# Jakoebly/marl-sc

Hardware: AMD Instinct MI355X
Metric: env-steps/sec (agents×envs×steps) at 1/2/4/8 MI355X; CPU ref same host (higher is better)
Workload: dtype int32 state, u64 PCG64, f64 rewards, f32 obs; 1 GPU; InventoryEnvironment.step x 32768 envs/GPU, 8 agents x 64 regions x 5 SKUs (BASELINE configs[2]; configs[3] when N>1); n_envs_per_gpu=32768, agents=8, regions=64, skus=5, episode_length=100, obs_dim_local=34, obs_normalization=meanstd_custom, parallelism=env-shard x1

## Files before the change

### marl-sc_amd/csrc/demand_v3.hip

```cpp
#include <hip/hip_runtime.h>

#include "demand_common.hpp"

namespace msc {

#ifdef MSC_PROF
__device__ unsigned long long g_prof_v3[8];
#endif

template <int K, int G, bool EA>
__global__ __launch_bounds__(BS * (1 + G)) __attribute__((amdgpu_waves_per_eu(MSC_DEM_WPE))) void demand_v3_kernel(
    const DevEnv* __restrict__ dp, EaLaunch ea) {
  const EnvConst& c = dp->c;
  const EnvState& s = dp->s;
  constexpr int NV = Rec<K>::NV;
  extern __shared__ __attribute__((aligned(16))) double v3lds[];
  __shared__ int more[2];
  double* ring = v3lds;
  int32_t* rdv = reinterpret_cast<int32_t*>(v3lds + BS * USLOTS);
  const int wave = (int)(threadIdx.x / BS), lane = (int)(threadIdx.x % BS);
  const int64_t E = c.E;
  const int64_t vlane = (int64_t)blockIdx.x * BS + lane;
  int64_t e = vlane;
  int slot = 0, ea_k = 0;
  bool valid = vlane < E;
  if constexpr (EA) {
    valid = vlane < (int64_t)ea.nslots * E;
    ea_k = valid ? (int)(vlane / E) : 0;
    e = valid ? vlane - (int64_t)ea_k * E : 0;
    slot = (ea.slot0 + ea_k) % c.ea_S;
  }
  double* myring = ring + lane;
  int ea_cnt_new = 0;
  uint32_t ea_p0 = 0;
  int ea_n0 = 0;
  if constexpr (EA) {
    if (valid && ea.t0 > 0) {
      ea_p0 = s.ea_pos[((int64_t)slot * c.T + (ea.t0 - 1)) * E + e];
      ea_n0 = s.ea_off[((int64_t)slot * (c.T + 1) + ea.t0) * E + e];
    }
  }
  auto start_rng = [&]() -> Pcg64 {
    if constexpr (EA) {
      uint32_t root;
      if (ea.t0 == 0) {
        root = ea_root(c, s, ea, e, ea_k, slot, ea_cnt_new);
      } else {
        const uint32_t w2[2] = {s.orig_root[e], (uint32_t)(s.ea_cnt[(int64_t)slot * E + e] - 1)};
        root = ss_u32(w2, 2);
      }
      Pcg64 r;
      pcg_seed_child(r, root, 2);
      if (ea_p0) pcg_advance(r, (uint64_t)ea_p0);
      return r;
    } else {
      return load_rng(s, 0, e, E);
    }
  };

  if (wave > 0) {
    if (MSC_GEN_PRIO > 0) __builtin_amdgcn_s_setprio(MSC_GEN_PRIO);
    const int g = wave - 1;
    uint64_t th = 0, tl = 0, ih = 0, il = 1;
    if (valid) {
      Pcg64 rg = start_rng();
      for (int j = 0; j <= g; j++) pcg_step(rg);
      th = rg.s_hi;
      tl = rg.s_lo;
      ih = rg.i_hi;
      il = rg.i_lo;
    }
    uint64_t mh = PCG_MUL_HI, ml = PCG_MUL_LO, ch = ih, cl = il;
    if constexpr (G > 1) pcg_jump_coeffs(G, ih, il, mh, ml, ch, cl);
    int pg = g;
    GenLane gl = gen_lane(th, tl, ch, cl);
    auto gen_to = [&](int target) {
      while (pg < target) {
        const double u = gen_uniform(gl);
        const int sl = pg & (UCAP - 1);
        myring[sl * BS] = u;
        myring[(sl < UD - 1 ? sl + UCAP : USLOTS - 1) * BS] = u;
        gen_advance<G>(gl);
        pg += G;
      }
    };
    int tgt = UCAP;
    if (valid) gen_to(UCAP);
    __syncthreads();
    for (int ci = 0;; ci++) {
      const int rdp = rdv[(ci & 1) * BS + lane];
      tgt = unit_quota(tgt, rdp);
      if (valid) gen_to(tgt);
      __syncthreads();
      if (!more[ci & 1]) break;
      const int need = rdv[((ci + 1) & 1) * BS + lane] + UHS * UD;
      if (__ballot(valid && tgt < need) != 0) {
        tgt = tgt > need ? tgt : need;
        if (valid) gen_to(tgt);
        __syncthreads();
      }
    }
    return;
  }

  __builtin_amdgcn_s_setprio(MSC_PARSER_PRIO);
  Pcg64 r0{};
  if (valid) {
    r0 = start_rng();
    if constexpr (!EA) store_rng_pre(s, e, E, r0);
  }
  rdv[lane] = 0;
  static_assert(K <= UD, "a mask unit completes in one round");
  int qf = 0, mf = 0, of = valid ? 1 : 0, live = of;
  int r = 0, x = 0, left = 0, sq = 0, n = ea_n0, rd = 0, pend = 0;
  int tstep = EA ? ea.t0 : 0;
  unsigned mask = 0;
  const int cap = EA ? (int)c.ea_cap : c.order_cap;
  const int64_t vstride = EA ? 16 : E * 16;
  const int64_t rstride = (int64_t)NV * vstride;
  MSC_GLOBAL char* const recb = reinterpret_cast<MSC_GLOBAL char*>(
      gp(EA ? s.ea_rec + ((int64_t)slot * E + e) * c.ea_cap * NV : s.orders + e));
  decltype(s.ea_off) ea_offp = EA ? s.ea_off + (int64_t)slot * (c.T + 1) * E + e : nullptr;
  decltype(s.ea_pos) ea_posp = EA ? s.ea_pos + (int64_t)slot * c.T * E + e : nullptr;
  const int T_s = __builtin_amdgcn_readfirstlane(EA ? ea.t1 : c.T);
  __syncthreads();
  if constexpr (EA) {
    if (valid && ea.t0 == 0) {
      s.ea_cnt[(int64_t)slot * E + e] = ea_cnt_new;
      ea_offp[0] = 0;
    }
  }
  double thr_o = sgpr_d(c.uni_thr_o), thr_q = sgpr_d(c.uni_thr_q);
  asm volatile("" : "+v"(thr_o), "+v"(thr_q));
  const double thr_m = sgpr_d(c.uni_thr_m);
  const int R_s = __builtin_amdgcn_readfirstlane(c.R), cap_s = __builtin_amdgcn_readfirstlane(cap);
  const uint32_t rs32 = (uint32_t)__builtin_amdgcn_readfirstlane((uint32_t)rstride);
  auto rec_at = [&](int idx) -> MSC_GLOBAL char* { return recb + (int64_t)((uint64_t)(uint32_t)idx * rs32); };
  int ridx = (n < cap_s ? n : cap_s) - 1;
  double thr = thr_o, prod = 1.0;
  auto settle = [&]() {
    if (qf) {
      const int h = 1 + sq;
      MSC_GLOBAL char* fp = NV == 1 ? rec_at(ridx) + h * 2 : rec_at(ridx) + (int64_t)(h >> 3) * vstride + (h & 7) * 2;
      *reinterpret_cast<MSC_GLOBAL uint16_t*>(fp) = (uint16_t)(x > 1 ? x : 1);
    }
    const unsigned m2 = qf ? (mask & (mask - 1u)) : mask;
    const int has_q = (of ^ 1) & (m2 != 0u ? 1 : 0);
    const int left2 = (of ? x : left) - ((of | has_q) ^ 1);
    const int new_order = (has_q ^ 1) & (left2 > 0 ? 1 : 0);
    const int new_region = (has_q | new_order) ^ 1;
    int wrap = 0;
    if constexpr (EA) {
      if (new_region & (r + 1 == R_s ? 1 : 0)) {
        ea_offp[(int64_t)(tstep + 1) * E] = n;
        ea_posp[(int64_t)tstep * E] = ea_p0 + (uint32_t)rd;
        wrap = tstep + 1 < T_s ? 1 : 0;
        tstep += wrap;
      }
    }
    sq = __builtin_ctz(m2 | (1u << K));
    qf = has_q;
    mf = new_order;
    of = new_region & ((r + 1 < R_s ? 1 : 0) | wrap);
    live = qf | mf | of;
    thr = has_q ? thr_q : thr_o;
    mask = new_order ? 0u : m2;
    left = left2;
    n += new_order;
    ridx = (n < cap_s ? n : cap_s) - 1;
    if (new_order) {
      MSC_GLOBAL char* rp = rec_at(ridx);
#pragma unroll
      for (int j = 0; j < NV; j++)
        *reinterpret_cast<MSC_GLOBAL v4u*>(rp + (int64_t)j * vstride) = v4u{j == 0 ? (unsigned)r : 0u, 0u, 0u, 0u};
    }
    r = wrap ? 0 : r + new_region;
    prod = 1.0;
    x = 0;
  };
#ifdef MSC_PROF
  unsigned long long n_round = 0;
#endif
  int ptgt = UCAP, rd_start = 0;
  for (int ci = 0;; ci++) {
#pragma unroll 1
    for (int hs = 0; hs < UHS; hs++) {
      const double* rp = myring + (rd & (UCAP - 1)) * BS;
      double u[UD];
#pragma unroll
      for (int i = 0; i < UD; i++) u[i] = rp[i * BS];
      if (pend) settle();
      double p = prod;
      int ncont = 0;
      unsigned bits = 0;
#pragma unroll
      for (int i = 0; i < UD; i++) {
        p = p * u[i];
        ncont += p > thr ? 1 : 0;
        if (i < K) bits |= u[i] > thr_m ? 0u : (1u << i);
      }
      const int go = ncont >= UD ? 1 : 0;
      const int cons = mf ? K : (go ? UD : ncont + 1);
      mask = mf ? bits : mask;
      x += ncont;
      prod = p;
      rd += live ? cons : 0;
      pend = live & (mf | (go ^ 1));
#ifdef MSC_PROF
      n_round++;
#endif
    }
    const bool any = __ballot(live) != 0;
    rdv[((ci + 1) & 1) * BS + lane] = rd;
    if (lane == 0) more[ci & 1] = any ? 1 : 0;
    __syncthreads();
    if (!any) break;
    ptgt = unit_quota(ptgt, rd_start);
    const int need = rd + UHS * UD;
    if (__ballot(valid && ptgt < need) != 0) {
      ptgt = ptgt > need ? ptgt : need;
      __syncthreads();
    }
    rd_start = rd;
  }
#ifdef MSC_PROF
  if (lane == 0) {
    atomicAdd(&g_prof_v3[0], n_round);
    atomicAdd(&g_prof_v3[2], 1ull);
  }
#endif
  if (!valid) return;
  if constexpr (EA) {
    if (n > cap) atomicOr(s.err, ERR_ORDER_OVERFLOW);
    return;
  }
  pcg_advance(r0, (uint64_t)rd);
  store_rng(s, 0, e, E, r0);
  if (n > cap) {
    atomicOr(s.err, ERR_ORDER_OVERFLOW);
    n = cap;
  }
  s.n_orders[e] = n;
}

bool demand_v3_supported(const EnvConst& c) {
  return c.demand_uni != 0 && c.demand_ptrs == 0 && c.K >= 1 && c.K <= UD && c.K <= 8 &&
         (uint64_t)c.E * 32u < (1ull << 32);
}

template <int K>
static void launch_v3_k(const EnvConst& c, const DevEnv* d, hipStream_t st, const EaLaunch* ea) {
  constexpr int G = 3;
  if (ea) {
    hipLaunchKernelGGL((demand_v3_kernel<K, G, true>), dim3((unsigned)(((int64_t)ea->nslots * c.E + BS - 1) / BS)),
                       dim3(BS * (1 + G)), unit_lds_fixed(), st, d, *ea);
  } else {
    hipLaunchKernelGGL((demand_v3_kernel<K, G, false>), dim3((unsigned)((c.E + BS - 1) / BS)), dim3(BS * (1 + G)),
                       unit_lds_fixed(), st, d, EaLaunch{0, 0, 0, 0, 0, 0, 0});
  }
}

hipError_t launch_demand_v3(const EnvConst& c, const DevEnv* d, hipStream_t st, const EaLaunch* ea) {
  switch (c.K) {
    case 1: launch_v3_k<1>(c, d, st, ea); break;
    case 2: launch_v3_k<2>(c, d, st, ea); break;
    case 3: launch_v3_k<3>(c, d, st, ea); break;
    case 4: launch_v3_k<4>(c, d, st, ea); break;
    case 5: launch_v3_k<5>(c, d, st, ea); break;
    case 6: launch_v3_k<6>(c, d, st, ea); break;
    case 7: launch_v3_k<7>(c, d, st, ea); break;
    case 8: launch_v3_k<8>(c, d, st, ea); break;
    default: return hipErrorInvalidValue;
  }
  return hipGetLastError();
}

template <int G>
__global__ __launch_bounds__(BS) void gen_draws_kernel(const uint64_t* __restrict__ state, const uint64_t* __restrict__ inc,
                                                       int64_t n, uint64_t* __restrict__ out,
                                                       uint64_t* __restrict__ state_out) {
  if (blockIdx.x != 0) return;
  const int lane = (int)threadIdx.x;
  GenLane gl = gen_lane(state[2 * lane], state[2 * lane + 1], inc[2 * lane], inc[2 * lane + 1]);
  for (int64_t i = 0; i < n; i++) {
    out[(int64_t)lane * n + i] = (uint64_t)__double_as_longlong(gen_uniform(gl));
    gen_advance<G>(gl);
  }
  state_out[2 * lane] = gen_state_hi(gl);
  state_out[2 * lane + 1] = gen_state_lo(gl);
}

hipError_t launch_gen_draws(int G, const uint64_t* state, const uint64_t* inc, int64_t n, uint64_t* out,
                            uint64_t* state_out, hipStream_t st) {
  switch (G) {
    case 1: hipLaunchKernelGGL(gen_draws_kernel<1>, dim3(1), dim3(BS), 0, st, state, inc, n, out, state_out); break;
    case 2: hipLaunchKernelGGL(gen_draws_kernel<2>, dim3(1), dim3(BS), 0, st, state, inc, n, out, state_out); break;
    case 3: hipLaunchKernelGGL(gen_draws_kernel<3>, dim3(1), dim3(BS), 0, st, state, inc, n, out, state_out); break;
    case 5: hipLaunchKernelGGL(gen_draws_kernel<5>, dim3(1), dim3(BS), 0, st, state, inc, n, out, state_out); break;
    case 7: hipLaunchKernelGGL(gen_draws_kernel<7>, dim3(1), dim3(BS), 0, st, state, inc, n, out, state_out); break;
    default: return hipErrorInvalidValue;
  }
  return hipGetLastError();
}

#ifdef MSC_PROF
extern "C" int msc_debug_prof_v3(unsigned long long* out, int reset) {
  if (hipMemcpyFromSymbol(out, HIP_SYMBOL(g_prof_v3), sizeof(unsigned long long) * 8) != hipSuccess) return -1;
  if (reset) {
    unsigned long long z[8] = {};
    if (hipMemcpyToSymbol(HIP_SYMBOL(g_prof_v3), z, sizeof z) != hipSuccess) return -1;
  }
  return 0;
}
#endif

}
```

Baseline: 369.1 million agent-steps/s.

## Replace demand-v3 catch-up barrier with fixed per-round generator quota and stall flag

Removes the conditional second __syncthreads round in both the generator and parser waves, where generators topped up the ring whenever any lane's parser needed more uniforms. Generators now produce a fixed quota per round (MSC_V3_QUOTA, a multiple of G=3, capped by ring capacity), and a parser lane skips its round when its lookahead is not yet covered. This cuts per-round barriers and ballots, but lanes that outrun the quota stall for a round, which may add rounds for fast-consuming lanes. Profiling counters for passes, draws and throttled rounds are added under MSC_PROF.

```diff
diff --git a/marl-sc_amd/csrc/demand_v3.hip b/marl-sc_amd/csrc/demand_v3.hip
--- a/marl-sc_amd/csrc/demand_v3.hip
+++ b/marl-sc_amd/csrc/demand_v3.hip
@@ -7,6 +7,19 @@
 #ifdef MSC_PROF
 __device__ unsigned long long g_prof_v3[8];
 #endif
+
+#ifndef MSC_V3_QUOTA
+#define MSC_V3_QUOTA 21
+#endif
+#ifndef MSC_V3_QUOTA_ODD
+#define MSC_V3_QUOTA_ODD MSC_V3_QUOTA
+#endif
+static_assert(MSC_V3_QUOTA > 0 && MSC_V3_QUOTA % 3 == 0 && MSC_V3_QUOTA_ODD > 0 && MSC_V3_QUOTA_ODD % 3 == 0,
+              "whole generator passes (G = 3)");
+__device__ __forceinline__ int v3_quota(int tgt, int rdp, int ci) {
+  const int q = tgt + ((ci & 1) ? MSC_V3_QUOTA_ODD : MSC_V3_QUOTA), cap = rdp + UCAP;
+  return q < cap ? q : cap;
+}
 
 template <int K, int G, bool EA>
 __global__ __launch_bounds__(BS * (1 + G)) __attribute__((amdgpu_waves_per_eu(MSC_DEM_WPE))) void demand_v3_kernel(
@@ -74,7 +87,20 @@
     if constexpr (G > 1) pcg_jump_coeffs(G, ih, il, mh, ml, ch, cl);
     int pg = g;
     GenLane gl = gen_lane(th, tl, ch, cl);
+#ifdef MSC_PROF
+    unsigned long long n_pass = 0, n_draw = 0;
+#endif
     auto gen_to = [&](int target) {
+#ifdef MSC_PROF
+      int it = valid && pg < target ? (target - pg + G - 1) / G : 0;
+      n_draw += (unsigned long long)it;
+      for (int o = BS / 2; o > 0; o >>= 1) {
+        const int other = __shfl_xor(it, o, BS);
+        it = it > other ? it : other;
+      }
+      n_pass += (unsigned long long)it;
+#endif
+      if (!valid) return;
       while (pg < target) {
         const double u = gen_uniform(gl);
         const int sl = pg & (UCAP - 1);
@@ -85,21 +111,19 @@
       }
     };
     int tgt = UCAP;
-    if (valid) gen_to(UCAP);
+    gen_to(UCAP);
     __syncthreads();
     for (int ci = 0;; ci++) {
       const int rdp = rdv[(ci & 1) * BS + lane];
-      tgt = unit_quota(tgt, rdp);
-      if (valid) gen_to(tgt);
+      tgt = v3_quota(tgt, rdp, ci);
+      gen_to(tgt);
       __syncthreads();
       if (!more[ci & 1]) break;
-      const int need = rdv[((ci + 1) & 1) * BS + lane] + UHS * UD;
-      if (__ballot(valid && tgt < need) != 0) {
-        tgt = tgt > need ? tgt : need;
-        if (valid) gen_to(tgt);
-        __syncthreads();
-      }
-    }
+    }
+#ifdef MSC_PROF
+    if (lane == 0) atomicAdd(&g_prof_v3[4], n_pass);
+    if (n_draw) atomicAdd(&g_prof_v3[5], n_draw);
+#endif
     return;
   }
 
@@ -179,48 +203,48 @@
     x = 0;
   };
 #ifdef MSC_PROF
-  unsigned long long n_round = 0;
+  unsigned long long n_round = 0, n_thr = 0;
 #endif
   int ptgt = UCAP, rd_start = 0;
+  bool ok = true;
   for (int ci = 0;; ci++) {
+#ifdef MSC_PROF
+    n_round += __ballot(ok) != 0 ? UHS : 0;
+    n_thr += !ok && live ? 1 : 0;
+#endif
+    if (ok) {
 #pragma unroll 1
-    for (int hs = 0; hs < UHS; hs++) {
-      const double* rp = myring + (rd & (UCAP - 1)) * BS;
-      double u[UD];
+      for (int hs = 0; hs < UHS; hs++) {
+        const double* rp = myring + (rd & (UCAP - 1)) * BS;
+        double u[UD];
 #pragma unroll
-      for (int i = 0; i < UD; i++) u[i] = rp[i * BS];
-      if (pend) settle();
-      double p = prod;
-      int ncont = 0;
-      unsigned bits = 0;
+        for (int i = 0; i < UD; i++) u[i] = rp[i * BS];
+        if (pend) settle();
+        double p = prod;
+        int ncont = 0;
+        unsigned bits = 0;
 #pragma unroll
-      for (int i = 0; i < UD; i++) {
-        p = p * u[i];
-        ncont += p > thr ? 1 : 0;
-        if (i < K) bits |= u[i] > thr_m ? 0u : (1u << i);
-      }
-      const int go = ncont >= UD ? 1 : 0;
-      const int cons = mf ? K : (go ? UD : ncont + 1);
-      mask = mf ? bits : mask;
-      x += ncont;
-      prod = p;
-      rd += live ? cons : 0;
-      pend = live & (mf | (go ^ 1));
-#ifdef MSC_PROF
-      n_round++;
-#endif
+        for (int i = 0; i < UD; i++) {
+          p = p * u[i];
+          ncont += p > thr ? 1 : 0;
+          if (i < K) bits |= u[i] > thr_m ? 0u : (1u << i);
+        }
+        const int go = ncont >= UD ? 1 : 0;
+        const int cons = mf ? K : (go ? UD : ncont + 1);
+        mask = mf ? bits : mask;
+        x += ncont;
+        prod = p;
+        rd += live ? cons : 0;
+        pend = live & (mf | (go ^ 1));
+      }
     }
     const bool any = __ballot(live) != 0;
     rdv[((ci + 1) & 1) * BS + lane] = rd;
     if (lane == 0) more[ci & 1] = any ? 1 : 0;
     __syncthreads();
     if (!any) break;
-    ptgt = unit_quota(ptgt, rd_start);
-    const int need = rd + UHS * UD;
-    if (__ballot(valid && ptgt < need) != 0) {
-      ptgt = ptgt > need ? ptgt : need;
-      __syncthreads();
-    }
+    ptgt = v3_quota(ptgt, rd_start, ci);
+    ok = ptgt >= rd + UHS * UD;
     rd_start = rd;
   }
 #ifdef MSC_PROF
@@ -228,6 +252,7 @@
     atomicAdd(&g_prof_v3[0], n_round);
     atomicAdd(&g_prof_v3[2], 1ull);
   }
+  if (n_thr) atomicAdd(&g_prof_v3[3], n_thr);
 #endif
   if (!valid) return;
   if constexpr (EA) {
```

Measured after the change: 378.3 million agent-steps/s, median of 6. +2.5%, better.
